# Fil/nd4js

Hardware: AMD Instinct MI355X
Metric: fp64 GFLOP/s: matmul N=4096 & SVD N=2048; % of MFMA/HBM peak (higher is better)
Workload: dtype f64; 1 GPU; matmul 4096x4096x4096 fp64, one matrix pair per GPU (BASELINE configs[1]); parallelism=batch-sharded x1, no collective, inputs=uniform(-1,1) seeds 5/6, HBM-resident

## Files before the change

### nd4js_amd/csrc/svd_block.hip

```cpp
#include "svd_internal.h"
#include <cstdlib>

typedef double d4 __attribute__((ext_vector_type(4)));
typedef double d2 __attribute__((ext_vector_type(2)));

namespace {

constexpr int BB = 32;
constexpr int PB = 64;
constexpr int CH = 256;

template <int K> __device__ __forceinline__ int bcast_i(int v) { return __builtin_amdgcn_readlane(v, K); }
template <int K> __device__ __forceinline__ double bcast_d(double v) {
  return __hiloint2double(__builtin_amdgcn_readlane(__double2hiint(v), K), __builtin_amdgcn_readlane(__double2loint(v), K));
}

__device__ __forceinline__ double fast_rcp(double x) {
  double r = __builtin_amdgcn_rcp(x);
  r = fma(fma(-x, r, 1.0), r, r);
  r = fma(fma(-x, r, 1.0), r, r);
  return r;
}
__device__ __forceinline__ double fast_rsqrt(double x) {
  double r = __builtin_amdgcn_rsq(x);
  r = r * fma(-0.5 * x * r, r, 1.5);
  r = r * fma(-0.5 * x * r, r, 1.5);
  return r;
}

__device__ __forceinline__ long pair_row(int x, int I, int J) { return x < BB ? (long)I * BB + x : (long)J * BB + (x - BB); }

__host__ __device__ __forceinline__ void jacb_pair(int n2, int s, int i, int& I, int& J) {
  if (n2 > 0) { nd4_rr_pair(n2, s, i, I, J); return; }
  const int n = -n2, h = n / 2, q = n / 4;
  const int grp = i >= q ? 1 : 0, ii = i - grp * q;
  if (s < h - 1) {
    nd4_rr_pair(h, s, ii, I, J);
    I += grp * h; J += grp * h;
  } else {
    const int c = s - (h - 1), second = c >= q ? 1 : 0, cc = c - second * q;
    I = grp * q + ii;
    J = h + ((grp ^ second) ? q : 0) + (ii + cc) % q;
  }
}
__host__ __device__ __forceinline__ int jacb_abs(int n2) { return n2 < 0 ? -n2 : n2; }

__device__ __forceinline__ void gram_load_group(d2 (&dst)[2][4], const double* const (&rp)[4], int c) {
#pragma unroll
  for (int t = 0; t < 4; t++) {
    dst[0][t] = *reinterpret_cast<const d2*>(rp[t] + c);
    dst[1][t] = *reinterpret_cast<const d2*>(rp[t] + c + 2);
  }
}
__device__ __forceinline__ void gram_mfma_group(d4 (&acc)[4][4], const d2 (&f)[2][4]) {
#pragma unroll
  for (int u = 0; u < 2; u++)
#pragma unroll
    for (int i = 0; i < 4; i++)
#pragma unroll
      for (int j = i; j < 4; j++) {
        acc[i][j] = __builtin_amdgcn_mfma_f64_16x16x4f64(f[u][i].x, f[u][j].x, acc[i][j], 0, 0, 0);
        acc[i][j] = __builtin_amdgcn_mfma_f64_16x16x4f64(f[u][i].y, f[u][j].y, acc[i][j], 0, 0, 0);
      }
}
__device__ __forceinline__ void gram_accumulate(d4 (&acc)[4][4], const double* const (&rp)[4], int col0, int ncols, int N, int fk) {
  for (int c0 = col0; c0 < col0 + ncols && c0 < N; c0 += 16) {
    d2 f[2][4];
    gram_load_group(f, rp, c0 + 4 * fk);
    gram_mfma_group(acc, f);
  }
}
template <int LDG>
__device__ __forceinline__ void gram_reduce_lds(double (*G)[LDG], const d4 (&acc)[4][4], int wave, int fk, int fx) {
#pragma unroll
  for (int w = 0; w < 4; w++) {
    if (wave == w) {
#pragma unroll
      for (int i = 0; i < 4; i++)
#pragma unroll
        for (int j = i; j < 4; j++)
#pragma unroll
          for (int r = 0; r < 4; r++) {
            const int row = i * 16 + fk + 4 * r, col = j * 16 + fx;
            double* d = &G[row][col];
            const double v = (w == 0) ? acc[i][j][r] : *d + acc[i][j][r];
            *d = v;
            if (w == 3 && j > i) G[col][row] = v;
          }
    }
    __syncthreads();
  }
}

template <int NT>
__device__ __forceinline__ void gram2_tiles(d4 (&acc)[3], const double (*st)[PB + 2], const int (&ti)[3], const int (&tj)[3], int fx, int fk) {
#pragma unroll
  for (int ks = 0; ks < 16; ks++) {
    double f[4];
#pragma unroll
    for (int q = 0; q < 4; q++) f[q] = st[q * 16 + fx][ks * 4 + fk];
#pragma unroll
    for (int n = 0; n < NT; n++) acc[n] = __builtin_amdgcn_mfma_f64_16x16x4f64(f[ti[n]], f[tj[n]], acc[n], 0, 0, 0);
  }
}
__global__ __launch_bounds__(256) void jacb_gram2(const double* __restrict__ Wm, int N, long sM, int nblk, int nblk2, int step,
                                                   const JacState* __restrict__ st, double* __restrict__ Gpart, int nchunks, long sG_mat, int pair0) {
  __shared__ double s_x[2][PB][PB + 2];
  const int pairIdx = blockIdx.x + pair0, chunk = blockIdx.y, mat = blockIdx.z;
  if (st[mat].done) return;
  int I, J;
  jacb_pair(nblk2, step, pairIdx, I, J);
  if (J >= nblk) return;
  const double* W = Wm + mat * sM;
  const int t = threadIdx.x, lane = t & 63, wave = __builtin_amdgcn_readfirstlane(t >> 6);
  const int fx = lane & 15, fk = lane >> 4;
  const double* src[8];
#pragma unroll
  for (int k = 0; k < 8; k++) src[k] = W + pair_row((t >> 5) + 8 * k, I, J) * N + chunk * CH + 2 * (t & 31);
  const int nsub = (N - chunk * CH >= CH) ? CH / 64 : (N - chunk * CH) / 64;
  d2 v[8];
  auto load = [&](int sub) {
#pragma unroll
    for (int k = 0; k < 8; k++) v[k] = *reinterpret_cast<const d2*>(src[k] + sub * 64);
  };
  auto stash = [&](int buf) {
#pragma unroll
    for (int k = 0; k < 8; k++) *reinterpret_cast<d2*>(&s_x[buf][(t >> 5) + 8 * k][2 * (t & 31)]) = v[k];
  };
  d4 acc[3] = {d4{0.0, 0.0, 0.0, 0.0}, d4{0.0, 0.0, 0.0, 0.0}, d4{0.0, 0.0, 0.0, 0.0}};
  if (nsub > 0) { load(0); stash(0); }
  __syncthreads();
  for (int sub = 0; sub < nsub; sub++) {
    if (sub + 1 < nsub) load(sub + 1);
    const double (*sx)[PB + 2] = s_x[sub & 1];
    if (wave == 0)      { const int ti[3] = {0, 0, 0}, tj[3] = {0, 1, 2}; gram2_tiles<3>(acc, sx, ti, tj, fx, fk); }
    else if (wave == 1) { const int ti[3] = {0, 1, 1}, tj[3] = {3, 1, 2}; gram2_tiles<3>(acc, sx, ti, tj, fx, fk); }
    else if (wave == 2) { const int ti[3] = {1, 2, 2}, tj[3] = {3, 2, 2}; gram2_tiles<2>(acc, sx, ti, tj, fx, fk); }
    else                { const int ti[3] = {2, 3, 3}, tj[3] = {3, 3, 3}; gram2_tiles<2>(acc, sx, ti, tj, fx, fk); }
    if (sub + 1 < nsub) stash((sub + 1) & 1);
    __syncthreads();
  }
  const int TI[4][3] = {{0, 0, 0}, {0, 1, 1}, {1, 2, 2}, {2, 3, 3}};
  const int TJ[4][3] = {{0, 1, 2}, {3, 1, 2}, {3, 2, 2}, {3, 3, 3}};
  double* G = Gpart + mat * sG_mat + ((long)pairIdx * nchunks + chunk) * (PB * PB);
  const int ntiles = wave < 2 ? 3 : 2;
#pragma unroll
  for (int n = 0; n < 3; n++) {
    if (n < ntiles) {
      const int i = TI[wave][n], j = TJ[wave][n];
#pragma unroll
      for (int r = 0; r < 4; r++) G[(i * 16 + fk + 4 * r) * PB + j * 16 + fx] = acc[n][r];
    }
  }
}

template <bool FUSED, int PW>
__global__ __launch_bounds__(2048 / PW) void jacb_eigen(const double* __restrict__ Gpart, int nchunks, long sG_mat, int nblk, int nblk2, int step,
                                                   JacState* __restrict__ st, const double* __restrict__ floor2, double tol2,
                                                   double* __restrict__ Qt_all, long sQ_mat, int* __restrict__ flags, long sF_mat,
                                                   unsigned long long* __restrict__ offmax, int max_inner, int cross_only) {
  __shared__ double G[PB][PB + 1];
  __shared__ double Q[PB][PB + 1];
  __shared__ unsigned s_rot[32 / PW];
  const int pairIdx = blockIdx.x, mat = blockIdx.y;
  if (st[mat].done) return;
  int I, J;
  jacb_pair(nblk2, step, pairIdx, I, J);
  if (J >= nblk) return;
  const int t = threadIdx.x, lane = t & 63, wave = t >> 6;
  if constexpr (FUSED) {
    static_assert(!FUSED || PW == 8, "the fused Gram phase is written for 4 waves");
    const int N = nchunks, fx = lane & 15, fk = lane >> 4;
    const double* W = Gpart + mat * sG_mat;
    const double* rp[4];
#pragma unroll
    for (int q = 0; q < 4; q++) rp[q] = W + pair_row(q * 16 + fx, I, J) * N;
    d4 acc[4][4];
#pragma unroll
    for (int i = 0; i < 4; i++)
#pragma unroll
      for (int j = 0; j < 4; j++) acc[i][j] = d4{0.0, 0.0, 0.0, 0.0};
    const int per = ((N + 63) / 64) * 16;
    gram_accumulate(acc, rp, wave * per, per, N, fk);
    gram_reduce_lds<PB + 1>(G, acc, wave, fk, fx);
    for (int e = t; e < PB * PB; e += 2048 / PW) Q[e / PB][e % PB] = (e / PB == e % PB) ? 1.0 : 0.0;
  } else {
    const double* Gp = Gpart + mat * sG_mat + (long)pairIdx * nchunks * (PB * PB);
    for (int e = t; e < PB * PB; e += 2048 / PW) {
      const int r = e / PB, c = e % PB;
      Q[r][c] = (r == c) ? 1.0 : 0.0;
      if ((r >> 4) > (c >> 4)) continue;
      double s = 0.0;
      for (int ch = 0; ch < nchunks; ch++) s += Gp[(long)ch * (PB * PB) + e];
      G[r][c] = s;
      if ((r >> 4) != (c >> 4)) G[c][r] = s;
    }
  }
  __syncthreads();
  const double fl = floor2[mat];
  unsigned total = 0;
  double relmax = 0.0;
  {
    int need = 0;
    for (int e = t; e < PB * PB; e += 2048 / PW) {
      const int i = e / PB, j = e % PB;
      if (i < j) { const double a = G[i][i], b = G[j][j], g = G[i][j]; need |= (a > fl) && (b > fl) && (g * g > tol2 * a * b); }
    }
    need = __syncthreads_or(need);
    if (!need) { if (t == 0) flags[mat * sF_mat + pairIdx] = 0; return; }
  }
  const int nrounds = cross_only ? BB : PB - 1;
  for (int inner = 0; inner < max_inner; inner++) {
    unsigned rot = 0;
    for (int r = 0; r < nrounds; r++) {
      int p, q;
      if (cross_only) { p = wave * PW + (lane & (PW - 1)); q = BB + ((p + r) & (BB - 1)); }
      else nd4_rr_pair(PB, r, wave * PW + (lane & (PW - 1)), p, q);
      const double a = G[p][p], b = G[q][q], g = G[p][q];
      const bool go = (a > fl) && (b > fl) && (g * g > tol2 * a * b);
      double c = 1.0, s = 0.0;
      if (go) {
        const double d = b - a, hh = 2.0 * g, rr = d * d + hh * hh;
        const double root = rr * fast_rsqrt(rr);
        const double tn = (((d < 0.0) != (g < 0.0)) ? -fabs(hh) : fabs(hh)) * fast_rcp(fabs(d) + root);
        const double cc = fast_rsqrt(1.0 + tn * tn);
        s = cc * tn;
        c = s * fast_rcp(1.0 + cc);
        relmax = fmax(relmax, (g * g) / (a * b));
      }
      rot += (unsigned)__popcll(__ballot(go && lane < PW));
      double sk[PW], ck[PW]; int pk[PW], qk[PW];
#define ND4_BC(K) sk[K] = bcast_d<K>(s); ck[K] = bcast_d<K>(c); pk[K] = bcast_i<K>(p); qk[K] = bcast_i<K>(q);
      ND4_BC(0) ND4_BC(1)
      if constexpr (PW > 2) { ND4_BC(2) ND4_BC(3) }
      if constexpr (PW > 4) { ND4_BC(4) ND4_BC(5) ND4_BC(6) ND4_BC(7) }
#undef ND4_BC
      {
        double gp[PW], gq[PW], up[PW], uq[PW];
#pragma unroll
        for (int k = 0; k < PW; k++) { gp[k] = G[pk[k]][lane]; gq[k] = G[qk[k]][lane]; up[k] = Q[pk[k]][lane]; uq[k] = Q[qk[k]][lane]; }
#pragma unroll
        for (int k = 0; k < PW; k++) {
          G[pk[k]][lane] = gp[k] - sk[k] * (gq[k] + ck[k] * gp[k]);
          G[qk[k]][lane] = gq[k] + sk[k] * (gp[k] - ck[k] * gq[k]);
          Q[pk[k]][lane] = up[k] - sk[k] * (uq[k] + ck[k] * up[k]);
          Q[qk[k]][lane] = uq[k] + sk[k] * (up[k] - ck[k] * uq[k]);
        }
      }
      __syncthreads();
      {
        double gp[PW], gq[PW];
#pragma unroll
        for (int k = 0; k < PW; k++) { gp[k] = G[lane][pk[k]]; gq[k] = G[lane][qk[k]]; }
#pragma unroll
        for (int k = 0; k < PW; k++) {
          G[lane][pk[k]] = gp[k] - sk[k] * (gq[k] + ck[k] * gp[k]);
          G[lane][qk[k]] = gq[k] + sk[k] * (gp[k] - ck[k] * gq[k]);
        }
      }
      __syncthreads();
    }
    if (lane == 0) s_rot[wave] = rot;
    __syncthreads();
    unsigned tot = 0;
    for (int w = 0; w < 32 / PW; w++) tot += s_rot[w];
    __syncthreads();
    total += tot;
    if (tot == 0) break;
  }
  double* Qt = Qt_all + mat * sQ_mat + (long)pairIdx * (PB * PB);
  if (total) for (int e = t; e < PB * PB; e += 2048 / PW) Qt[e] = Q[e / PB][e % PB];
#pragma unroll
  for (int off = 32; off > 0; off >>= 1) relmax = fmax(relmax, __shfl_xor(relmax, off));
  if (lane == 0 && relmax > 0.0) atomicMax(offmax, (unsigned long long)__double_as_longlong(relmax));
  if (t == 0) {
    flags[mat * sF_mat + pairIdx] = total ? 1 : 0;
    if (total) atomicAdd(&st[mat].rotations, total);
  }
}

template <int CG>
__device__ __forceinline__ void eigen_p_body(double* __restrict__ stage_raw, const int pairIdx, const int mat,
                                             const double* __restrict__ Gpart, int nchunks, long sG_mat, int nblk, int nblk2, int step,
                                             JacState* __restrict__ st, const double* __restrict__ floor2, double tol2,
                                             double* __restrict__ Qt_all, long sQ_mat, int* __restrict__ flags, long sF_mat,
                                             unsigned long long* __restrict__ offmax, int precheck) {
  constexpr int T = 576, TB = 512, NB = 2, NQ = 4;
  constexpr int LD = BB + 1;
  __shared__ double sC[2][BB][LD];
  __shared__ double sB[2][BB][LD];
  __shared__ double sA1[2][BB];
  __shared__ double sAng[2][2][BB];
  double (*stage)[PB + 1] = reinterpret_cast<double (*)[PB + 1]>(stage_raw);
  __shared__ double sRd[PB];
  __shared__ unsigned sTotal;
  double (*QJ)[PB + 1] = stage;
  if (st[mat].done) return;
  int I, J;
  jacb_pair(nblk2, step, pairIdx, I, J);
  if (J >= nblk) return;
  const int t = threadIdx.x, lane = t & 63, wave = t >> 6;
  if (t < TB) {
    constexpr int KL = (PB * PB / 2) / TB;
    const d2* Gp = reinterpret_cast<const d2*>(Gpart + mat * sG_mat + (long)pairIdx * nchunks * (PB * PB));
    d2 acc[KL];
#pragma unroll
    for (int k = 0; k < KL; k++) acc[k] = d2{0.0, 0.0};
    for (int ch0 = 0; ch0 < nchunks; ch0 += CG) {
      d2 v[CG][KL];
#pragma unroll
      for (int c = 0; c < CG; c++)
#pragma unroll
        for (int k = 0; k < KL; k++) {
          const int e = 2 * (t + TB * k);
          v[c][k] = (ch0 + c < nchunks && ((e / PB) >> 4) <= ((e % PB) >> 4)) ? Gp[(long)(ch0 + c) * (PB * PB / 2) + t + TB * k] : d2{0.0, 0.0};
        }
#pragma unroll
      for (int c = 0; c < CG; c++)
#pragma unroll
        for (int k = 0; k < KL; k++) acc[k] += v[c][k];
    }
#pragma unroll
    for (int k = 0; k < KL; k++) {
      const int e = 2 * (t + TB * k), r = e / PB, c = e % PB;
      if ((r >> 4) <= (c >> 4)) {
        stage[r][c] = acc[k].x;
        stage[r][c + 1] = acc[k].y;
        if ((r >> 4) != (c >> 4)) { stage[c][r] = acc[k].x; stage[c + 1][r] = acc[k].y; }
      }
    }
  }
  __syncthreads();
  const double fl = floor2[mat];
  if (precheck) {
    if (t < PB) { const double dd = stage[t][t]; sRd[t] = dd > fl ? __builtin_amdgcn_rcp(dd) : 0.0; }
    __syncthreads();
    double rel = 0.0;
    for (int e = t; e < PB * PB; e += T) {
      const int x = e / PB, y = e % PB;
      const double g = stage[x][y];
      if (x < y) rel = fmax(rel, g * g * sRd[x] * sRd[y]);
    }
#pragma unroll
    for (int off = 32; off > 0; off >>= 1) rel = fmax(rel, __shfl_xor(rel, off));
    if (lane == 0 && rel > 0.0) atomicMax(offmax, (unsigned long long)__double_as_longlong(rel));
    const int need = __syncthreads_or(rel > tol2 * (1.0 - 0x1p-20));
    if (!need) { if (t == 0) flags[mat * sF_mat + pairIdx] = 0; return; }
  }
  const int i = lane & 31, h = lane >> 5;
  const bool pivot = wave == 8;
  const int jb = NB * (2 * wave + h);
  const int cb = NQ * (2 * wave + h);
  double Areg[NB] = {0.0, 0.0}, Qp[NQ] = {0.0, 0.0, 0.0, 0.0};
  double pa = 0.0, pb = 0.0, pg = 0.0;
  if (pivot) {
    pa = stage[i][i]; pb = stage[BB + i][BB + i]; pg = stage[i][BB + i];
  } else {
#pragma unroll
    for (int m = 0; m < NB; m++) Areg[m] = stage[i][jb + m];
#pragma unroll
    for (int m = 0; m < NQ; m++) Qp[m] = (cb + m == i) ? 1.0 : 0.0;
  }
  for (int e = t; e < BB * BB; e += T) {
    const int x = e / BB, y = e % BB;
    sC[0][x][y] = stage[x][BB + y];
    sB[0][x][y] = stage[BB + x][BB + y];
  }
  if (t < BB) sA1[0][t] = stage[t][(t + 1) & (BB - 1)];
  __syncthreads();
  for (int e = t; e < BB * PB; e += T) QJ[e / PB][e % PB] = (e % PB == BB + e / PB) ? 1.0 : 0.0;
  unsigned rot = 0;
  double ps = 0.0, ptau = 0.0, sn = 0.0, tn = 0.0;
  for (int k = 0; k <= BB; k++) {
    const int prv = (k + 1) & 1, cur = k & 1;
    if (pivot) {
      if (k > 0) {
        const int ipp = (i + k - 1) & (BB - 1), y = (i + k) & (BB - 1), i1 = (i + 1) & (BB - 1);
        const double xpp = sA1[prv][i], xpq = sC[prv][i][y], xqp = sC[prv][i1][ipp], xqq = sB[prv][ipp][y];
        const double ypq = xpq - ps * (xqq + ptau * xpq), ypp = xpp - ps * (xqp + ptau * xpp);
        pg = ypq + sn * (ypp - tn * ypq);
      }
      if (k < BB) {
        const double a = pa, b = pb, g = pg;
        const bool go = (a > fl) && (b > fl) && (g * g > tol2 * a * b);
        const double d = b - a, hh = g + g, rr = fma(d, d, hh * hh);
        const double rs = fast_rsqrt(rr);
        const double x = fma(0.5 * fabs(d), rs, 0.5);
        const double ric = fast_rsqrt(x);
        const double c = x * ric;
        const double sabs = fabs(g) * rs * ric;
        double s = ((d < 0.0) != (g < 0.0)) ? -sabs : sabs;
        double tau = s * fast_rcp(1.0 + c);
        double tt = s * ric;
        if (!go) { s = 0.0; tau = 0.0; tt = 0.0; }
        rot += (unsigned)__popc((unsigned)__ballot(go));
        ps = s; ptau = tau;
        if (h == 0) { sAng[cur][0][i] = s; sAng[cur][1][i] = tau; }
        const int i1 = (i + 1) & (BB - 1);
        pa = a - tt * g;
        pb = __shfl(b + tt * g, i1);
        sn = __shfl(s, i1); tn = __shfl(tau, i1);
      }
    } else if (k > 0) {
      const int r = k - 1;
      const int ip = (i + r) & (BB - 1);
      const double s = sAng[prv][0][i], tau = sAng[prv][1][i];
      double xpq[NB], xqp[NB], xqq[NB], sjv[NB], tjv[NB], uq[NQ];
      int jp[NB];
#pragma unroll
      for (int m = 0; m < NB; m++) {
        jp[m] = (jb + m + r) & (BB - 1);
        xpq[m] = sC[prv][i][jp[m]];
        xqp[m] = sC[prv][jb + m][ip];
        xqq[m] = sB[prv][ip][jp[m]];
        sjv[m] = sAng[prv][0][jb + m];
        tjv[m] = sAng[prv][1][jb + m];
      }
#pragma unroll
      for (int m = 0; m < NQ; m++) uq[m] = QJ[ip][cb + m];
#pragma unroll
      for (int m = 0; m < NB; m++) {
        const double sj = sjv[m], tj = tjv[m];
        const double xpp = Areg[m];
        const double ypp = xpp - s * (xqp[m] + tau * xpp), yqp = xqp[m] + s * (xpp - tau * xqp[m]);
        const double ypq = xpq[m] - s * (xqq[m] + tau * xpq[m]), yqq = xqq[m] + s * (xpq[m] - tau * xqq[m]);
        const double zpp = ypp - sj * (ypq + tj * ypp);
        const double zpq = ypq + sj * (ypp - tj * ypq);
        const double zqq = yqq + sj * (yqp - tj * yqq);
        Areg[m] = zpp;
        if (jb + m == ((i + 1) & (BB - 1))) sA1[cur][i] = zpp;
        sC[cur][i][jp[m]] = zpq;
        sB[cur][ip][jp[m]] = zqq;
      }
#pragma unroll
      for (int m = 0; m < NQ; m++) {
        const double up = Qp[m];
        Qp[m] = up - s * (uq[m] + tau * up);
        QJ[ip][cb + m] = uq[m] + s * (up - tau * uq[m]);
      }
    }
    __syncthreads();
  }
  if (t == 8 * 64) sTotal = rot;
  __syncthreads();
  const unsigned total = sTotal;
  if (total) {
    double* Qt = Qt_all + mat * sQ_mat + (long)pairIdx * (PB * PB);
    if (!pivot) {
#pragma unroll
      for (int m = 0; m < NQ; m++) Qt[i * PB + cb + m] = Qp[m];
    }
    for (int e = t; e < BB * PB; e += T) Qt[BB * PB + e] = QJ[e / PB][e % PB];
  }
  if (t == 0) {
    flags[mat * sF_mat + pairIdx] = total ? 1 : 0;
    if (total) atomicAdd(&st[mat].rotations, total);
  }
}

constexpr int SQ_LD = PB + 4;
constexpr int STAGE_DOUBLES = PB * SQ_LD;
template <int T, int STRIPS = 4>
__device__ __forceinline__ void apply_body(double* __restrict__ sq_raw, const int pairIdx, int chunk, const int mat,
                                           double* __restrict__ Wm, double* __restrict__ Utm, int N, long sM, int nblk, int nblk2, int step,
                                           const JacState* __restrict__ st, const double* __restrict__ Qt_all, long sQ_mat,
                                           const int* __restrict__ flags, long sF_mat, int nchunks) {
  double (*sQ)[SQ_LD] = reinterpret_cast<double (*)[SQ_LD]>(sq_raw);
  if (st[mat].done || !flags[mat * sF_mat + pairIdx]) return;
  int I, J;
  jacb_pair(nblk2, step, pairIdx, I, J);
  if (J >= nblk) return;
  double* X = (chunk < nchunks ? Wm : Utm) + mat * sM;
  if (chunk >= nchunks) chunk -= nchunks;
  const int t = threadIdx.x, lane = t & 63, wave = t >> 6;
  const int fx = lane & 15, fk = lane >> 4;
  const double* Qt = Qt_all + mat * sQ_mat + (long)pairIdx * (PB * PB);
  for (int e = t; e < PB * PB; e += T) sQ[e / PB][e % PB] = Qt[e];
  __syncthreads();
  if (T > 256 && t >= 256) return;
  long rowoff[16];
#pragma unroll
  for (int ks = 0; ks < 16; ks++) rowoff[ks] = pair_row(ks * 4 + fk, I, J) * N;
  const int colw = chunk * (64 * STRIPS) + wave * (16 * STRIPS);
  for (int strip = 0; strip < STRIPS; strip++) {
    const int cbase = colw + strip * 16;
    if (cbase >= N) break;
    const int c = cbase + fx;
    double b[16];
#pragma unroll
    for (int ks = 0; ks < 16; ks++) b[ks] = X[rowoff[ks] + c];
#pragma unroll
    for (int it = 0; it < 4; it++) {
      d4 acc = d4{0.0, 0.0, 0.0, 0.0};
#pragma unroll
      for (int ks = 0; ks < 16; ks++)
        acc = __builtin_amdgcn_mfma_f64_16x16x4f64(sQ[it * 16 + fx][ks * 4 + fk], b[ks], acc, 0, 0, 0);
#pragma unroll
      for (int r = 0; r < 4; r++) X[pair_row(it * 16 + fk + 4 * r, I, J) * N + c] = acc[r];
    }
  }
}

__global__ __launch_bounds__(576) void jacb_eigen_p(const double* __restrict__ Gpart, int nchunks, long sG_mat, int nblk, int nblk2, int step,
                                                     JacState* __restrict__ st, const double* __restrict__ floor2, double tol2,
                                                     double* __restrict__ Qt_all, long sQ_mat, int* __restrict__ flags, long sF_mat,
                                                     unsigned long long* __restrict__ offmax, int precheck, int pair0) {
  __shared__ double stage_raw[STAGE_DOUBLES];
  eigen_p_body<4>(stage_raw, blockIdx.x + pair0, blockIdx.y, Gpart, nchunks, sG_mat, nblk, nblk2, step, st, floor2, tol2, Qt_all, sQ_mat, flags, sF_mat,
               offmax, precheck);
}

__global__ __launch_bounds__(256) void jacb_apply(double* __restrict__ Wm, double* __restrict__ Utm, int N, long sM, int nblk, int nblk2, int step,
                                                   const JacState* __restrict__ st, const double* __restrict__ Qt_all, long sQ_mat,
                                                   const int* __restrict__ flags, long sF_mat, int nchunks, int chunk0, int pair0) {
  __shared__ double sq_raw[STAGE_DOUBLES];
  apply_body<256>(sq_raw, blockIdx.x + pair0, blockIdx.y + chunk0, blockIdx.z, Wm, Utm, N, sM, nblk, nblk2, step, st, Qt_all, sQ_mat, flags, sF_mat, nchunks);
}

template <int STRIPS>
__global__ __launch_bounds__(256) void jacb_apply_w(double* __restrict__ Wm, int N, long sM, int nblk, int nblk2, int step,
                                                     const JacState* __restrict__ st, const double* __restrict__ Qt_all, long sQ_mat,
                                                     const int* __restrict__ flags, long sF_mat, int pair0) {
  __shared__ double sq_raw[STAGE_DOUBLES];
  apply_body<256, STRIPS>(sq_raw, blockIdx.x + pair0, blockIdx.y, blockIdx.z, Wm, nullptr, N, sM, nblk, nblk2, step, st, Qt_all, sQ_mat, flags, sF_mat,
                          (int)gridDim.y);
}

__global__ __launch_bounds__(576) void jacb_eigen_pu(const double* __restrict__ Gpart, int nchunks, long sG_mat, int nblk, int nblk2, int step,
                                                      JacState* __restrict__ st, const double* __restrict__ floor2, double tol2,
                                                      double* __restrict__ Qt_all, long sQ_mat, int* __restrict__ flags, long sF_mat,
                                                      unsigned long long* __restrict__ offmax, int precheck, int npairs,
                                                      double* __restrict__ Utm, int N, long sM, const double* __restrict__ Qt_prev,
                                                      const int* __restrict__ flags_prev, int pair0) {
  __shared__ double stage_raw[STAGE_DOUBLES];
  if ((int)blockIdx.x < npairs) {
    eigen_p_body<8>(stage_raw, blockIdx.x + pair0, blockIdx.y, Gpart, nchunks, sG_mat, nblk, nblk2, step, st, floor2, tol2, Qt_all, sQ_mat, flags, sF_mat,
                 offmax, precheck);
  } else {
    const int idx = (int)blockIdx.x - npairs;
    apply_body<576>(stage_raw, idx % npairs + pair0, nchunks + idx / npairs, blockIdx.y, nullptr, Utm, N, sM, nblk, nblk2, step - 1, st, Qt_prev, sQ_mat,
                    flags_prev, sF_mat, nchunks);
  }
}

}

size_t nd4_jacobi_block_scratch_doubles(int batch, int N) {
  const int nblk = N / BB, nblk2 = (nblk + 1) & ~1, npairs = nblk2 / 2, nchunks = (N + CH - 1) / CH;
  const size_t per = (size_t)npairs * nchunks * PB * PB + 2 * ((size_t)npairs * PB * PB + (size_t)((npairs + 1) / 2 + 1));
  return per * batch;
}

namespace {

struct JacbSweep {
  nd4hip_handle* h;
  int batch, N; double* W; double* Ut; JacState* st; const double* floor2; double tol2; unsigned long long* offmax;
  int precheck;
  int nblk, npairs, nchunks;
  long sM, sG, sQ, sF;
  double* Gpart; double* Qt2[2]; int* flags2[2];
  int wstrips;
};

void jacb_launch_apply_w(const JacbSweep& s, hipStream_t stream, int n2, int step, int np, int batch, double* Qt, int* flags, int p0) {
  if (s.wstrips == 1)
    hipLaunchKernelGGL(jacb_apply_w<1>, dim3((unsigned)np, (unsigned)(s.N / 64), (unsigned)batch), dim3(256), 0, stream,
                       s.W, s.N, s.sM, s.nblk, n2, step, s.st, Qt, s.sQ, flags, s.sF, p0);
  else
    hipLaunchKernelGGL(jacb_apply_w<2>, dim3((unsigned)np, (unsigned)((s.N + 127) / 128), (unsigned)batch), dim3(256), 0, stream,
                       s.W, s.N, s.sM, s.nblk, n2, step, s.st, Qt, s.sQ, flags, s.sF, p0);
}

int jacb_sweep_two_chains(const JacbSweep& s) {
  nd4hip_handle* h = s.h;
  const int N = s.N, nblk = s.nblk, npairs = s.npairs, nchunks = s.nchunks;
  const int n2 = -nblk, hq = nblk / 2, q = nblk / 4, nsteps = nblk - 1;
  hipStream_t chain[2] = {h->stream, h->aux_stream};
  hipLaunchKernelGGL(jacb_gram2, dim3((unsigned)npairs, (unsigned)nchunks, 1u), dim3(256), 0, chain[0], s.W, N, s.sM, nblk, n2, 0, s.st, s.Gpart, nchunks, s.sG, 0);
  hipLaunchKernelGGL((jacb_eigen<false, 2>), dim3((unsigned)npairs, 1u), dim3(1024), 0, chain[0],
                     s.Gpart, nchunks, s.sG, nblk, n2, 0, s.st, s.floor2, s.tol2, s.Qt2[0], s.sQ, s.flags2[0], s.sF, s.offmax, 1, 0);
  hipLaunchKernelGGL(jacb_apply, dim3((unsigned)npairs, (unsigned)(2 * nchunks), 1u), dim3(256), 0, chain[0],
                     s.W, s.Ut, N, s.sM, nblk, n2, 0, s.st, s.Qt2[0], s.sQ, s.flags2[0], s.sF, nchunks, 0, 0);
  ND4_HIP(hipEventRecord(h->ev_aux_a, chain[0]));
  ND4_HIP(hipStreamWaitEvent(chain[1], h->ev_aux_a, 0));
  bool prev_full = true;
  for (int step = 1; step < nsteps; step++) {
    const bool phase_end = step == hq - 2 || step == hq - 2 + q || step == nsteps - 1;
    double* Qt = s.Qt2[step & 1];
    int* flags = s.flags2[step & 1];
    for (int c = 0; c < 2; c++) {
      const int p0 = c * q;
      hipLaunchKernelGGL(jacb_gram2, dim3((unsigned)q, (unsigned)nchunks, 1u), dim3(256), 0, chain[c], s.W, N, s.sM, nblk, n2, step, s.st, s.Gpart, nchunks, s.sG, p0);
      if (prev_full)
        hipLaunchKernelGGL(jacb_eigen_p, dim3((unsigned)q, 1u), dim3(576), 0, chain[c],
                           s.Gpart, nchunks, s.sG, nblk, n2, step, s.st, s.floor2, s.tol2, Qt, s.sQ, flags, s.sF, s.offmax, s.precheck, p0);
      else
        hipLaunchKernelGGL(jacb_eigen_pu, dim3((unsigned)(q + q * nchunks), 1u), dim3(576), 0, chain[c],
                           s.Gpart, nchunks, s.sG, nblk, n2, step, s.st, s.floor2, s.tol2, Qt, s.sQ, flags, s.sF, s.offmax, s.precheck, q,
                           s.Ut, N, s.sM, s.Qt2[(step - 1) & 1], s.flags2[(step - 1) & 1], p0);
      if (phase_end)
        hipLaunchKernelGGL(jacb_apply, dim3((unsigned)q, (unsigned)(2 * nchunks), 1u), dim3(256), 0, chain[c],
                           s.W, s.Ut, N, s.sM, nblk, n2, step, s.st, Qt, s.sQ, flags, s.sF, nchunks, 0, p0);
      else
        jacb_launch_apply_w(s, chain[c], n2, step, q, 1, Qt, flags, p0);
    }
    prev_full = phase_end;
    if (phase_end) {
      ND4_HIP(hipEventRecord(h->ev_aux_a, chain[0]));
      ND4_HIP(hipEventRecord(h->ev_aux_b, chain[1]));
      ND4_HIP(hipStreamWaitEvent(chain[1], h->ev_aux_a, 0));
      ND4_HIP(hipStreamWaitEvent(chain[0], h->ev_aux_b, 0));
    }
  }
  ND4_HIP(hipGetLastError());
  return 0;
}

int jacb_sweep_one_chain(const JacbSweep& s, const bool defer) {
  nd4hip_handle* h = s.h;
  const int N = s.N, batch = s.batch, nblk = s.nblk, nblk2 = (nblk + 1) & ~1, npairs = s.npairs, nchunks = s.nchunks;
  const bool fused = N <= 1024 && batch * npairs >= 128 && batch * npairs <= 768;
  for (int step = 0; step < nblk2 - 1; step++) {
    const bool cross_only = step > 0;
    double* Qt = s.Qt2[defer ? (step & 1) : 0];
    int* flags = s.flags2[defer ? (step & 1) : 0];
    const bool last = step == nblk2 - 2;
    if (fused) {
      hipLaunchKernelGGL((jacb_eigen<true, 8>), dim3((unsigned)npairs, (unsigned)batch), dim3(256), 0, h->stream,
                         s.W, N, s.sM, nblk, nblk2, step, s.st, s.floor2, s.tol2, Qt, s.sQ, flags, s.sF, s.offmax, 1, cross_only ? 1 : 0);
    } else {
      hipLaunchKernelGGL(jacb_gram2, dim3((unsigned)npairs, (unsigned)nchunks, (unsigned)batch), dim3(256), 0, h->stream,
                         s.W, N, s.sM, nblk, nblk2, step, s.st, s.Gpart, nchunks, s.sG, 0);
      if (cross_only && defer) {
        hipLaunchKernelGGL(jacb_eigen_pu, dim3((unsigned)(npairs + npairs * nchunks), (unsigned)batch), dim3(576), 0, h->stream,
                           s.Gpart, nchunks, s.sG, nblk, nblk2, step, s.st, s.floor2, s.tol2, Qt, s.sQ, flags, s.sF, s.offmax, s.precheck, npairs,
                           s.Ut, N, s.sM, s.Qt2[(step - 1) & 1], s.flags2[(step - 1) & 1], 0);
      } else if (cross_only) {
        hipLaunchKernelGGL(jacb_eigen_p, dim3((unsigned)npairs, (unsigned)batch), dim3(576), 0, h->stream,
                           s.Gpart, nchunks, s.sG, nblk, nblk2, step, s.st, s.floor2, s.tol2, Qt, s.sQ, flags, s.sF, s.offmax, s.precheck, 0);
      } else if ((long)batch * npairs <= 256) {
        hipLaunchKernelGGL((jacb_eigen<false, 2>), dim3((unsigned)npairs, (unsigned)batch), dim3(1024), 0, h->stream,
                           s.Gpart, nchunks, s.sG, nblk, nblk2, step, s.st, s.floor2, s.tol2, Qt, s.sQ, flags, s.sF, s.offmax, 1, 0);
      } else {
        hipLaunchKernelGGL((jacb_eigen<false, 8>), dim3((unsigned)npairs, (unsigned)batch), dim3(256), 0, h->stream,
                           s.Gpart, nchunks, s.sG, nblk, nblk2, step, s.st, s.floor2, s.tol2, Qt, s.sQ, flags, s.sF, s.offmax, 1, 0);
      }
    }
    if (defer && !last)
      jacb_launch_apply_w(s, h->stream, nblk2, step, npairs, batch, Qt, flags, 0);
    else
      hipLaunchKernelGGL(jacb_apply, dim3((unsigned)npairs, (unsigned)(2 * nchunks), (unsigned)batch), dim3(256), 0, h->stream,
                         s.W, s.Ut, N, s.sM, nblk, nblk2, step, s.st, Qt, s.sQ, flags, s.sF, nchunks, 0, 0);
  }
  ND4_HIP(hipGetLastError());
  return 0;
}

}

int nd4_jacobi_block_sweep(nd4hip_handle* h, int batch, int N, double* W, double* Ut, JacState* st,
                           const double* floor2, double tol2, unsigned long long* offmax, double* scratch, bool dense_phase) {
  JacbSweep s;
  s.h = h; s.batch = batch; s.N = N; s.W = W; s.Ut = Ut; s.st = st; s.floor2 = floor2; s.tol2 = tol2; s.offmax = offmax;
  s.precheck = dense_phase ? 0 : 1;
  s.nblk = N / BB; s.npairs = ((s.nblk + 1) & ~1) / 2; s.nchunks = (N + CH - 1) / CH;
  s.sM = (long)N * N;
  s.sG = (long)s.npairs * s.nchunks * PB * PB; s.sQ = (long)s.npairs * PB * PB;
  s.sF = ((s.npairs + 1) / 2 + 1) * 2;
  s.Gpart = scratch;
  s.Qt2[0] = s.Gpart + (size_t)batch * s.sG;
  s.flags2[0] = reinterpret_cast<int*>(s.Qt2[0] + (size_t)batch * s.sQ);
  s.Qt2[1] = s.Qt2[0] + (size_t)batch * s.sQ + (size_t)batch * (s.sF / 2);
  s.flags2[1] = reinterpret_cast<int*>(s.Qt2[1] + (size_t)batch * s.sQ);
  s.wstrips = N <= 2048 ? 1 : 2;
  const bool defer = (long)batch * s.npairs <= 64 && N >= 512;
  const char* two_e = getenv("ND4HIP_JAC_TWO_CHAINS");
  const int two_min_n = two_e ? atoi(two_e) : 4096;
  if (two_min_n > 0 && defer && batch == 1 && s.nblk % 4 == 0 && N >= two_min_n) return jacb_sweep_two_chains(s);
  return jacb_sweep_one_chain(s, defer);
}
```

Measured before the change: 76270 GFLOP/s.

## Rewrite W-apply kernel with register-held operands and defer done-check past loads

Replaces the generic apply_body-based W update with a dedicated kernel. It loads the pair's rotation block and the W rows into registers, stores a permuted Qt image in shared memory, and issues paired MFMAs over 128-column chunks, so the old 1- and 2-strip variants are no longer needed. In the deferred and two-chain paths, the gram and eigen kernels now issue their global loads before checking the convergence flag, so the flag read no longer stalls the memory traffic. The cost is loads wasted on blocks that exit early, plus a new indexing scheme in apply_w that could be wrong.

```diff
diff --git a/nd4js_amd/csrc/svd_block.hip b/nd4js_amd/csrc/svd_block.hip
--- a/nd4js_amd/csrc/svd_block.hip
+++ b/nd4js_amd/csrc/svd_block.hip
@@ -103,11 +103,13 @@
     for (int n = 0; n < NT; n++) acc[n] = __builtin_amdgcn_mfma_f64_16x16x4f64(f[ti[n]], f[tj[n]], acc[n], 0, 0, 0);
   }
 }
+template <bool EARLY>
 __global__ __launch_bounds__(256) void jacb_gram2(const double* __restrict__ Wm, int N, long sM, int nblk, int nblk2, int step,
                                                    const JacState* __restrict__ st, double* __restrict__ Gpart, int nchunks, long sG_mat, int pair0) {
   __shared__ double s_x[2][PB][PB + 2];
   const int pairIdx = blockIdx.x + pair0, chunk = blockIdx.y, mat = blockIdx.z;
-  if (st[mat].done) return;
+  const int done = st[mat].done;
+  if (!EARLY && done) return;
   int I, J;
   jacb_pair(nblk2, step, pairIdx, I, J);
   if (J >= nblk) return;
@@ -130,6 +132,7 @@
   d4 acc[3] = {d4{0.0, 0.0, 0.0, 0.0}, d4{0.0, 0.0, 0.0, 0.0}, d4{0.0, 0.0, 0.0, 0.0}};
   if (nsub > 0) { load(0); stash(0); }
   __syncthreads();
+  if (EARLY && done) return;
   for (int sub = 0; sub < nsub; sub++) {
     if (sub + 1 < nsub) load(sub + 1);
     const double (*sx)[PB + 2] = s_x[sub & 1];
@@ -279,7 +282,7 @@
   }
 }
 
-template <int CG>
+template <int CG, bool EARLY>
 __device__ __forceinline__ void eigen_p_body(double* __restrict__ stage_raw, const int pairIdx, const int mat,
                                              const double* __restrict__ Gpart, int nchunks, long sG_mat, int nblk, int nblk2, int step,
                                              JacState* __restrict__ st, const double* __restrict__ floor2, double tol2,
@@ -295,7 +298,10 @@
   __shared__ double sRd[PB];
   __shared__ unsigned sTotal;
   double (*QJ)[PB + 1] = stage;
-  if (st[mat].done) return;
+  const int done = st[mat].done;
+  double fl = 0.0;
+  if constexpr (EARLY) fl = floor2[mat];
+  if (!EARLY && done) return;
   int I, J;
   jacb_pair(nblk2, step, pairIdx, I, J);
   if (J >= nblk) return;
@@ -331,7 +337,8 @@
     }
   }
   __syncthreads();
-  const double fl = floor2[mat];
+  if (EARLY && done) return;
+  if constexpr (!EARLY) fl = floor2[mat];
   if (precheck) {
     if (t < PB) { const double dd = stage[t][t]; sRd[t] = dd > fl ? __builtin_amdgcn_rcp(dd) : 0.0; }
     __syncthreads();
@@ -460,7 +467,7 @@
 
 constexpr int SQ_LD = PB + 4;
 constexpr int STAGE_DOUBLES = PB * SQ_LD;
-template <int T, int STRIPS = 4>
+template <int T>
 __device__ __forceinline__ void apply_body(double* __restrict__ sq_raw, const int pairIdx, int chunk, const int mat,
                                            double* __restrict__ Wm, double* __restrict__ Utm, int N, long sM, int nblk, int nblk2, int step,
                                            const JacState* __restrict__ st, const double* __restrict__ Qt_all, long sQ_mat,
@@ -478,6 +485,7 @@
   for (int e = t; e < PB * PB; e += T) sQ[e / PB][e % PB] = Qt[e];
   __syncthreads();
   if (T > 256 && t >= 256) return;
+  constexpr int STRIPS = 4;
   long rowoff[16];
 #pragma unroll
   for (int ks = 0; ks < 16; ks++) rowoff[ks] = pair_row(ks * 4 + fk, I, J) * N;
@@ -506,7 +514,7 @@
                                                      double* __restrict__ Qt_all, long sQ_mat, int* __restrict__ flags, long sF_mat,
                                                      unsigned long long* __restrict__ offmax, int precheck, int pair0) {
   __shared__ double stage_raw[STAGE_DOUBLES];
-  eigen_p_body<4>(stage_raw, blockIdx.x + pair0, blockIdx.y, Gpart, nchunks, sG_mat, nblk, nblk2, step, st, floor2, tol2, Qt_all, sQ_mat, flags, sF_mat,
+  eigen_p_body<4, false>(stage_raw, blockIdx.x + pair0, blockIdx.y, Gpart, nchunks, sG_mat, nblk, nblk2, step, st, floor2, tol2, Qt_all, sQ_mat, flags, sF_mat,
                offmax, precheck);
 }
 
@@ -517,13 +525,56 @@
   apply_body<256>(sq_raw, blockIdx.x + pair0, blockIdx.y + chunk0, blockIdx.z, Wm, Utm, N, sM, nblk, nblk2, step, st, Qt_all, sQ_mat, flags, sF_mat, nchunks);
 }
 
-template <int STRIPS>
+constexpr int WCH = 128;
+constexpr int SQW_LD = PB + 2;
+static_assert(PB * SQW_LD <= STAGE_DOUBLES, "the permuted Qt image fits the stage");
 __global__ __launch_bounds__(256) void jacb_apply_w(double* __restrict__ Wm, int N, long sM, int nblk, int nblk2, int step,
                                                      const JacState* __restrict__ st, const double* __restrict__ Qt_all, long sQ_mat,
                                                      const int* __restrict__ flags, long sF_mat, int pair0) {
-  __shared__ double sq_raw[STAGE_DOUBLES];
-  apply_body<256, STRIPS>(sq_raw, blockIdx.x + pair0, blockIdx.y, blockIdx.z, Wm, nullptr, N, sM, nblk, nblk2, step, st, Qt_all, sQ_mat, flags, sF_mat,
-                          (int)gridDim.y);
+  __shared__ double sq[PB * SQW_LD];
+  const int pairIdx = blockIdx.x + pair0, mat = blockIdx.z;
+  int I, J;
+  jacb_pair(nblk2, step, pairIdx, I, J);
+  if (J >= nblk) return;
+  const int t = threadIdx.x, lane = t & 63, wave = __builtin_amdgcn_readfirstlane(t >> 6);
+  const int fx = lane & 15, fk = lane >> 4;
+  const int done = st[mat].done, flag = flags[mat * sF_mat + pairIdx];
+  constexpr int KQ = PB * PB / 2 / 256;
+  const d2* Qt = reinterpret_cast<const d2*>(Qt_all + mat * sQ_mat + (long)pairIdx * (PB * PB));
+  d2 q[KQ];
+#pragma unroll
+  for (int k = 0; k < KQ; k++) q[k] = Qt[t + 256 * k];
+  double* X = Wm + mat * sM;
+  const int cw = (int)blockIdx.y * WCH + wave * 32;
+  const double* src = X + ((long)I * BB + fk) * N + (cw < N ? cw : 0) + 2 * fx;
+  const long jump = ((long)(J - I) * BB - BB) * N;
+  d2 b[16];
+#pragma unroll
+  for (int ks = 0; ks < 16; ks++) b[ks] = *reinterpret_cast<const d2*>(src + (long)(4 * ks) * N + (ks < 8 ? 0 : jump));
+#pragma unroll
+  for (int k = 0; k < KQ; k++) {
+    const int e = t + 256 * k;
+    double* d = sq + (e >> 5) * SQW_LD + (e & 1) * 16 + ((e & 31) >> 1);
+    d[0] = q[k].x;
+    d[32] = q[k].y;
+  }
+  __syncthreads();
+  if (done || !flag || cw >= N) return;
+#pragma unroll
+  for (int it = 0; it < 4; it++) {
+    d4 ae = d4{0.0, 0.0, 0.0, 0.0}, ao = d4{0.0, 0.0, 0.0, 0.0};
+#pragma unroll
+    for (int ks = 0; ks < 16; ks += 2) {
+      const d2 a = *reinterpret_cast<const d2*>(sq + (it * 16 + fx) * SQW_LD + ((fk & 1) * 2 + (fk >> 1)) * 16 + ks);
+      ae = __builtin_amdgcn_mfma_f64_16x16x4f64(a.x, b[ks].x, ae, 0, 0, 0);
+      ao = __builtin_amdgcn_mfma_f64_16x16x4f64(a.x, b[ks].y, ao, 0, 0, 0);
+      ae = __builtin_amdgcn_mfma_f64_16x16x4f64(a.y, b[ks + 1].x, ae, 0, 0, 0);
+      ao = __builtin_amdgcn_mfma_f64_16x16x4f64(a.y, b[ks + 1].y, ao, 0, 0, 0);
+    }
+#pragma unroll
+    for (int r = 0; r < 4; r++)
+      *reinterpret_cast<d2*>(X + pair_row(it * 16 + fk + 4 * r, I, J) * N + cw + 2 * fx) = d2{ae[r], ao[r]};
+  }
 }
 
 __global__ __launch_bounds__(576) void jacb_eigen_pu(const double* __restrict__ Gpart, int nchunks, long sG_mat, int nblk, int nblk2, int step,
@@ -534,7 +585,7 @@
                                                       const int* __restrict__ flags_prev, int pair0) {
   __shared__ double stage_raw[STAGE_DOUBLES];
   if ((int)blockIdx.x < npairs) {
-    eigen_p_body<8>(stage_raw, blockIdx.x + pair0, blockIdx.y, Gpart, nchunks, sG_mat, nblk, nblk2, step, st, floor2, tol2, Qt_all, sQ_mat, flags, sF_mat,
+    eigen_p_body<8, true>(stage_raw, blockIdx.x + pair0, blockIdx.y, Gpart, nchunks, sG_mat, nblk, nblk2, step, st, floor2, tol2, Qt_all, sQ_mat, flags, sF_mat,
                  offmax, precheck);
   } else {
     const int idx = (int)blockIdx.x - npairs;
@@ -560,16 +611,11 @@
   int nblk, npairs, nchunks;
   long sM, sG, sQ, sF;
   double* Gpart; double* Qt2[2]; int* flags2[2];
-  int wstrips;
 };
 
 void jacb_launch_apply_w(const JacbSweep& s, hipStream_t stream, int n2, int step, int np, int batch, double* Qt, int* flags, int p0) {
-  if (s.wstrips == 1)
-    hipLaunchKernelGGL(jacb_apply_w<1>, dim3((unsigned)np, (unsigned)(s.N / 64), (unsigned)batch), dim3(256), 0, stream,
-                       s.W, s.N, s.sM, s.nblk, n2, step, s.st, Qt, s.sQ, flags, s.sF, p0);
-  else
-    hipLaunchKernelGGL(jacb_apply_w<2>, dim3((unsigned)np, (unsigned)((s.N + 127) / 128), (unsigned)batch), dim3(256), 0, stream,
-                       s.W, s.N, s.sM, s.nblk, n2, step, s.st, Qt, s.sQ, flags, s.sF, p0);
+  hipLaunchKernelGGL(jacb_apply_w, dim3((unsigned)np, (unsigned)((s.N + WCH - 1) / WCH), (unsigned)batch), dim3(256), 0, stream,
+                     s.W, s.N, s.sM, s.nblk, n2, step, s.st, Qt, s.sQ, flags, s.sF, p0);
 }
 
 int jacb_sweep_two_chains(const JacbSweep& s) {
@@ -577,7 +623,7 @@
   const int N = s.N, nblk = s.nblk, npairs = s.npairs, nchunks = s.nchunks;
   const int n2 = -nblk, hq = nblk / 2, q = nblk / 4, nsteps = nblk - 1;
   hipStream_t chain[2] = {h->stream, h->aux_stream};
-  hipLaunchKernelGGL(jacb_gram2, dim3((unsigned)npairs, (unsigned)nchunks, 1u), dim3(256), 0, chain[0], s.W, N, s.sM, nblk, n2, 0, s.st, s.Gpart, nchunks, s.sG, 0);
+  hipLaunchKernelGGL(jacb_gram2<true>, dim3((unsigned)npairs, (unsigned)nchunks, 1u), dim3(256), 0, chain[0], s.W, N, s.sM, nblk, n2, 0, s.st, s.Gpart, nchunks, s.sG, 0);
   hipLaunchKernelGGL((jacb_eigen<false, 2>), dim3((unsigned)npairs, 1u), dim3(1024), 0, chain[0],
                      s.Gpart, nchunks, s.sG, nblk, n2, 0, s.st, s.floor2, s.tol2, s.Qt2[0], s.sQ, s.flags2[0], s.sF, s.offmax, 1, 0);
   hipLaunchKernelGGL(jacb_apply, dim3((unsigned)npairs, (unsigned)(2 * nchunks), 1u), dim3(256), 0, chain[0],
@@ -591,7 +637,7 @@
     int* flags = s.flags2[step & 1];
     for (int c = 0; c < 2; c++) {
       const int p0 = c * q;
-      hipLaunchKernelGGL(jacb_gram2, dim3((unsigned)q, (unsigned)nchunks, 1u), dim3(256), 0, chain[c], s.W, N, s.sM, nblk, n2, step, s.st, s.Gpart, nchunks, s.sG, p0);
+      hipLaunchKernelGGL(jacb_gram2<true>, dim3((unsigned)q, (unsigned)nchunks, 1u), dim3(256), 0, chain[c], s.W, N, s.sM, nblk, n2, step, s.st, s.Gpart, nchunks, s.sG, p0);
       if (prev_full)
         hipLaunchKernelGGL(jacb_eigen_p, dim3((unsigned)q, 1u), dim3(576), 0, chain[c],
                            s.Gpart, nchunks, s.sG, nblk, n2, step, s.st, s.floor2, s.tol2, Qt, s.sQ, flags, s.sF, s.offmax, s.precheck, p0);
@@ -630,7 +676,7 @@
       hipLaunchKernelGGL((jacb_eigen<true, 8>), dim3((unsigned)npairs, (unsigned)batch), dim3(256), 0, h->stream,
                          s.W, N, s.sM, nblk, nblk2, step, s.st, s.floor2, s.tol2, Qt, s.sQ, flags, s.sF, s.offmax, 1, cross_only ? 1 : 0);
     } else {
-      hipLaunchKernelGGL(jacb_gram2, dim3((unsigned)npairs, (unsigned)nchunks, (unsigned)batch), dim3(256), 0, h->stream,
+      hipLaunchKernelGGL(defer ? jacb_gram2<true> : jacb_gram2<false>, dim3((unsigned)npairs, (unsigned)nchunks, (unsigned)batch), dim3(256), 0, h->stream,
                          s.W, N, s.sM, nblk, nblk2, step, s.st, s.Gpart, nchunks, s.sG, 0);
       if (cross_only && defer) {
         hipLaunchKernelGGL(jacb_eigen_pu, dim3((unsigned)(npairs + npairs * nchunks), (unsigned)batch), dim3(576), 0, h->stream,
@@ -673,7 +719,6 @@
   s.flags2[0] = reinterpret_cast<int*>(s.Qt2[0] + (size_t)batch * s.sQ);
   s.Qt2[1] = s.Qt2[0] + (size_t)batch * s.sQ + (size_t)batch * (s.sF / 2);
   s.flags2[1] = reinterpret_cast<int*>(s.Qt2[1] + (size_t)batch * s.sQ);
-  s.wstrips = N <= 2048 ? 1 : 2;
   const bool defer = (long)batch * s.npairs <= 64 && N >= 512;
   const char* two_e = getenv("ND4HIP_JAC_TWO_CHAINS");
   const int two_min_n = two_e ? atoi(two_e) : 4096;
```

Result: no change. 76170 GFLOP/s (median of 2 runs) (-0.1%).
